# djukic14/BlockSparseMatrices.jl

Measured on AMD Instinct MI355X. Metric: fp64 block-SpMV GB/s (VBCRS mul!, algorithmic bytes / time), higher is better.
Workload: dtype f64

## Files before the change

### blocksparsematrices.jl_amd/csrc/bsm_analysis.cpp

```cpp
#include "bsm_analysis.h"

#include <algorithm>
#include <chrono>
#include <cstdio>
#include <cstdlib>
#include <cstring>
#include <numeric>
#include <set>
#include <thread>
#include <tuple>
#include <unordered_map>

namespace bsm {

Tunables Tunables::from_env() {
    Tunables t;
    auto geti = [](const char *name, int64_t dflt) -> int64_t {
        const char *s = std::getenv(name);
        if (!s || !*s) return dflt;
        return std::strtoll(s, nullptr, 10);
    };
    t.split2_bytes = geti("BSM_SPLIT2_BYTES", t.split2_bytes);
    t.split4_bytes = geti("BSM_SPLIT4_BYTES", t.split4_bytes);
    t.wgitem_max_bytes = geti("BSM_WGITEM_MAX_BYTES", t.wgitem_max_bytes);
    t.wave_bytes = geti("BSM_WAVE_BYTES", t.wave_bytes);
    t.multi_wave_bytes = geti("BSM_MULTI_WAVE_BYTES", t.multi_wave_bytes);
    t.target_waves = std::max<int64_t>(1, geti("BSM_TARGET_WAVES", t.target_waves));
    if (const char *f = std::getenv("BSM_FAT_FILL_BELOW")) t.fat_fill_below = std::atof(f);
    t.pack_threads = (int)geti("BSM_PACK_THREADS", t.pack_threads);
    t.wg_order = (int)geti("BSM_ORDER", t.wg_order);
    t.deep_group_bytes = geti("BSM_DEEP_GROUP_BYTES", t.deep_group_bytes);
    t.deep_total_bytes = geti("BSM_DEEP_TOTAL_BYTES", t.deep_total_bytes);
    t.window_bytes = (size_t)geti("BSM_UPLOAD_WINDOW_BYTES", (int64_t)t.window_bytes);
    if (t.pack_threads < 1) t.pack_threads = 1;
    return t;
}

namespace {

std::vector<std::vector<int32_t>> conflict_adjacency(const std::vector<const int64_t *> &lists,
                                                     const std::vector<int64_t> &lens) {
    const int64_t nb = (int64_t)lists.size();
    int64_t maxindex = 0;
    for (int64_t b = 0; b < nb; b++)
        for (int64_t k = 0; k < lens[b]; k++) maxindex = std::max(maxindex, lists[b][k]);
    std::vector<int64_t> ptr(maxindex + 2, 0);
    for (int64_t b = 0; b < nb; b++)
        for (int64_t k = 0; k < lens[b]; k++) ptr[lists[b][k] + 1]++;
    for (int64_t i = 0; i <= maxindex; i++) ptr[i + 1] += ptr[i];
    std::vector<int64_t> inc(ptr[maxindex + 1]);
    {
        std::vector<int64_t> fill(ptr.begin(), ptr.end() - 1);
        for (int64_t b = 0; b < nb; b++)
            for (int64_t k = 0; k < lens[b]; k++) inc[fill[lists[b][k]]++] = b;
    }
    std::vector<std::vector<int32_t>> adj(nb);
    std::vector<int64_t> stamp(nb, -1);
    for (int64_t v = 0; v < nb; v++) {
        stamp[v] = v;
        for (int64_t k = 0; k < lens[v]; k++) {
            int64_t i = lists[v][k];
            for (int64_t p = ptr[i]; p < ptr[i + 1]; p++) {
                int64_t w = inc[p];
// ... 204 lines not shown
        const int e_lo = (int)std::max<int64_t>(0, -w0);
        const int e_hi = (int)std::min<int64_t>(E, n - w0);
        U *d = dst + (s * mc) * E;
        if (!trans) {
            for (int e = e_lo; e < e_hi; e++) {
                const V *col = src + ra + (w0 + e) * ld;
                for (int i = 0; i < mc; i++) d[(int64_t)i * E + e] = stored(col[i]);
            }
        } else {
            for (int i = 0; i < mc; i++) {
                const V *row = src + w0 + (int64_t)(ra + i) * ld;
                for (int e = e_lo; e < e_hi; e++) d[(int64_t)i * E + e] = stored(row[e]);
            }
        }
    }
}

struct U16 {
    uint64_t a, b;
};

uint64_t hash_list(const int64_t *p, int64_t n) {
    uint64_t h = 0xcbf29ce484222325ull ^ (uint64_t)n;
    for (int64_t i = 0; i < n; i++) {
        h ^= (uint64_t)p[i];
        h *= 0x100000001b3ull;
        h ^= h >> 29;
    }
    return h;
}

}

struct Analysis::BuildState {
    bool sym = false;
    bool colored = false;
    int64_t nb = 0;
    int64_t own_lo = 0, own_hi = 0;
    std::vector<Chunk> chunks;
    std::vector<Group> groups;
    std::vector<const int64_t *> glist;
    std::vector<int32_t> colpos;
    std::vector<uint8_t> ckind;
    std::vector<uint8_t> group_perm;
    std::vector<int64_t> layout;
    uint64_t val_units = 0;
    std::vector<uint8_t> cover;
    std::vector<int32_t> group_color;
    int32_t ncolors_fused = 1;
    std::vector<Item> items;
    bool use_window = false;
};

std::string Analysis::build(int mtype_, int dtype_, int64_t nrows_, int64_t ncols_,
                            const std::vector<BlockIn> &blocks, const AnalysisOptions &opt_) {
    mtype = mtype_;
    dtype = dtype_;
    nrows = nrows_;
    ncols = ncols_;
    opt = opt_;
    tun = Tunables::from_env();
    const bool timing = std::getenv("BSM_TIMING") != nullptr;
    auto t_last = std::chrono::steady_clock::now();
    auto lap = [&](const char *what) {
        if (!timing) return;
        auto now = std::chrono::steady_clock::now();
        std::fprintf(stderr, "[bsm analysis] %-28s %8.1f ms\n", what,
                     std::chrono::duration<double, std::milli>(now - t_last).count());
        t_last = now;
    };
    BuildState st;
    std::string err = stage_validate(blocks, st);
    if (!err.empty()) return err;
    lap("validate");
    bool colour_oom = false;
    if (opt.meta_only) {
        reference_colourings(blocks, colour_oom);
        return colour_oom ? "out of host memory (colouring)" : "";
    }
    if (!(err = stage_row_groups(blocks, st)).empty()) return err;
    if (!(err = stage_merge_columns(blocks, st)).empty()) return err;
    lap("groups + column lists");
    if (!(err = stage_accumulation(blocks, st)).empty()) return err;
    lap("exclusivity / fused colours");
    std::thread colour_thread([&] { reference_colourings(blocks, colour_oom); });
    struct Joiner {
        std::thread &t;
        ~Joiner() {
            if (t.joinable()) t.join();
        }
    } colour_join{colour_thread};
    stage_work_items(st);
    stage_place_values(st);
    lap("work items + value placement");
    if (!(err = stage_pack_values(blocks, st)).empty()) return err;
    lap("pack values");
    stage_waves(st);
    stage_windows(st);
    if (!(err = stage_gather_index(st)).empty()) return err;
    lap("schedule");
    colour_thread.join();
    lap("reference colourings (tail not hidden by packing)");
    if (colour_oom) return "out of host memory (colouring)";
    return "";
}

std::string Analysis::stage_validate(const std::vector<BlockIn> &blocks, BuildState &st) {
    static const int kEs[6] = {4, 8, 8, 16, 4, 8};
    static const int kVs[6] = {4, 8, 8, 16, 8, 16};
    if (dtype < 0 || dtype > 5) return "unknown dtype";
    es = kEs[dtype];
    vs = kVs[dtype];
    E = 16 / es;
    if (nrows < 0 || ncols < 0) return "negative matrix size";
    if (nrows > INT32_MAX - 64 || ncols > INT32_MAX - 64) return "matrix dimension exceeds int32 range";
    const int64_t nb = st.nb = (int64_t)blocks.size();
    bool sym = (mtype == MT_SYMMETRIC);
    for (const BlockIn &B : blocks) sym |= (B.kind != KIND_PLAIN);
    st.sym = sym;
    st.own_lo = (opt.own_lo > 0) ? opt.own_lo - 1 : 0;
    st.own_hi = (opt.own_hi > 0) ? std::min(opt.own_hi, nrows) : nrows;
    const int64_t rlim = sym ? std::min(nrows, ncols) : nrows;
    const int64_t clim = sym ? std::min(nrows, ncols) : ncols;

    nnz = 0;
// ... 68 lines not shown
                }
            } else if (mtype == MT_SYMMETRIC) {
                std::vector<const int64_t *> dl, rl, cl;
                std::vector<int64_t> dn, rn, cn;
                for (const BlockIn &B : blocks) {
                    if (B.kind == KIND_DIAG) {
                        dl.push_back(B.ridx);
                        dn.push_back(B.ridx ? B.m : 0);
                    } else {
                        rl.push_back(B.ridx);
                        rn.push_back(B.ridx ? B.m : 0);
                        cl.push_back(B.cidx);
                        cn.push_back(B.cidx ? B.n : 0);
                    }
                }
                colors[0] = refcolor(rl, rn);
                colors[1] = refcolor(cl, cn);
                colors[2] = refcolor(dl, dn);
            }
        } catch (const std::bad_alloc &) {
            colour_oom = true;
        }
    }
}

std::string Analysis::stage_row_groups(const std::vector<BlockIn> &blocks, BuildState &st) {
    const int64_t nb = st.nb;
    auto &chunks = st.chunks;
    auto &groups = st.groups;
    auto &glist = st.glist;
    const int chunk_rows = tun.chunk_rows;
    std::unordered_map<uint64_t, std::vector<int64_t>> gmap;

    rows.clear();
    cols.clear();
    for (int64_t b = 0; b < nb; b++) {
        const BlockIn &B = blocks[b];
        if (B.m == 0 || B.n == 0) continue;
        for (int64_t ra = 0; ra < B.m; ra += chunk_rows) {
            const int mc = (int)std::min<int64_t>(chunk_rows, B.m - ra);
            bool rcontig = true;
            if (B.ridx)
                for (int i = 1; i < mc; i++)
                    if (B.ridx[ra + i] != B.ridx[ra] + i) {
                        rcontig = false;
                        break;
                    }
            const int64_t rbase = rcontig ? (B.ridx ? B.ridx[ra] : B.r0 + ra) - 1 : -1;
            uint64_t h;
            if (rcontig)
                h = ((uint64_t)rbase * 0x9E3779B97F4A7C15ull) ^ ((uint64_t)mc << 56) ^ 0x51ull;
            else
                h = hash_list(B.ridx + ra, mc);
            const int gkind = (B.kind == KIND_PLAIN) ? KIND_PLAIN : KIND_OFF;
            h ^= (uint64_t)gkind * 0xD6E8FEB86659FD93ull;
            int64_t gid = -1;
            auto &cand = gmap[h];
            for (int64_t g : cand) {
                const Group &G = groups[g];
                if (G.mc != mc || ((G.kind == KIND_PLAIN) != (B.kind == KIND_PLAIN))) continue;
                if (rcontig) {
                    if (G.rbase == rbase) gid = g;
                } else if (G.rbase < 0 &&
                           std::memcmp(glist[g], B.ridx + ra, sizeof(int64_t) * mc) == 0) {
                    gid = g;
                }
                if (gid >= 0) break;
            }
            if (gid < 0) {
                gid = (int64_t)groups.size();
                Group G;
                G.mc = mc;
                G.kind = B.kind;
                G.rbase = (int32_t)rbase;
                if (!rcontig) {
                    if ((int64_t)rows.size() + mc + 8 > INT32_MAX) return "row index pool exceeds int32";
                    G.row_off = (int32_t)rows.size();
                    for (int i = 0; i < mc; i++) rows.push_back((int32_t)(B.ridx[ra + i] - 1));
                }
                groups.push_back(G);
                glist.push_back(rcontig ? nullptr : B.ridx + ra);
                cand.push_back(gid);
            }
            Chunk c;
            c.blk = (int32_t)b;
            c.ra = (int32_t)ra;
            c.mc = mc;
            c.group = gid;
            c.woff = groups[gid].width;
            groups[gid].width += B.n;
            if (B.kind == KIND_OFF) {
                groups[gid].has_off = true;
                groups[gid].kind = KIND_OFF;
            } else if (B.kind == KIND_DIAG) {
                groups[gid].has_diag = true;
            }
            groups[gid].chunks.push_back((int32_t)chunks.size());
            chunks.push_back(c);
        }
    }
    ngroups = (int64_t)groups.size();
    return "";
}

std::string Analysis::stage_merge_columns(const std::vector<BlockIn> &blocks, BuildState &st) {
    auto &chunks = st.chunks;
    auto &groups = st.groups;
    auto &colpos = st.colpos;
    auto &ckind = st.ckind;
    auto &group_perm = st.group_perm;
    uint64_t val_units = 0;

    {
        int64_t total_cols = 0;
        for (const Group &G : groups) total_cols += G.width + E;
        if (total_cols + 8 > INT32_MAX) return "column index pool exceeds int32";
        cols.reserve((size_t)total_cols);
    }
    group_perm.assign(groups.size(), 0);
    colpos.reserve(cols.capacity());
    ckind.reserve(cols.capacity());
    {
        std::vector<int32_t> ord;
        size_t gi = 0;
        for (Group &G : groups) {
            G.strips = (G.width + E - 1) / E;
            if (G.strips * (int64_t)G.mc * 16 >= ((int64_t)1 << 31)) return "row group panel exceeds 2 GiB";
            G.col_off = (int64_t)cols.size();
            for (int32_t ci : G.chunks) {
                const BlockIn &B = blocks[chunks[ci].blk];
                for (int64_t k = 0; k < B.n; k++) {
                    cols.push_back((int32_t)((B.cidx ? B.cidx[k] : B.c0 + k) - 1));
                    ckind.push_back((uint8_t)B.kind);
                }
            }
            int32_t *gc = cols.data() + G.col_off;
            uint8_t *gk = ckind.data() + G.col_off;
            colpos.resize(cols.size());
            int32_t *gp = colpos.data() + G.col_off;
            if (std::is_sorted(gc, gc + G.width)) {
                for (int64_t q = 0; q < G.width; q++) gp[q] = (int32_t)q;
            } else {
                group_perm[gi] = 1;
                ord.resize((size_t)G.width);
                std::iota(ord.begin(), ord.end(), 0);
                std::stable_sort(ord.begin(), ord.end(), [&](int32_t a, int32_t b) { return gc[a] < gc[b]; });
                std::vector<int32_t> sorted((size_t)G.width);
                std::vector<uint8_t> sortedk((size_t)G.width);
                for (int64_t r = 0; r < G.width; r++) {
                    sorted[r] = gc[ord[r]];
                    sortedk[r] = gk[ord[r]];
                    gp[ord[r]] = (int32_t)r;
// ... 124 lines not shown
        if (tun.wgitem_max_bytes <= 0) tun.wgitem_max_bytes = 4 * W;
    }
    for (int64_t g = 0; g < ngroups; g++) {
        const Group &G = groups[g];
        const int64_t strip_bytes = (int64_t)G.mc * 16;
        int64_t per_item = G.strips;
        if (!exclusive_fwd && !colored) {
            int64_t maxs = std::max<int64_t>(1, tun.wgitem_max_bytes / strip_bytes);
            int64_t nitem = (G.strips + maxs - 1) / maxs;
            per_item = (G.strips + nitem - 1) / nitem;
        }
        for (int64_t s = 0; s < G.strips; s += per_item) {
            Item it;
            it.group = g;
            it.s_begin = s;
            it.s_end = std::min(G.strips, s + per_item);
            it.bytes = (it.s_end - it.s_begin) * strip_bytes;
            it.nw = it.bytes >= tun.split4_bytes ? 4 : (it.bytes >= tun.split2_bytes ? 2 : 1);
            it.color = group_color[g];
            items.push_back(it);
        }
    }
    const bool use_window = st.use_window = sym && !colored && !gather && !exclusive_fwd && tun.lds_window;
    auto locality = [&](const Item &it) -> int64_t {
        const Group &G = groups[it.group];
        return (G.rbase >= 0) ? G.rbase : rows[G.row_off];
    };
    std::stable_sort(items.begin(), items.end(), [&](const Item &a, const Item &b) {
        if (a.color != b.color) return a.color < b.color;
        if (a.nw != b.nw) return a.nw > b.nw;
        if (use_window && a.nw < 4) return locality(a) < locality(b);
        return a.bytes > b.bytes;
    });
}

void Analysis::stage_place_values(BuildState &st) {
    auto &groups = st.groups;
    std::vector<uint8_t> placed(groups.size(), 0);
    st.layout.clear();
    st.layout.reserve(groups.size());
    for (const Item &it : st.items)
        if (!placed[it.group]) {
            placed[it.group] = 1;
            st.layout.push_back(it.group);
        }
    for (size_t g = 0; g < groups.size(); g++)
        if (!placed[g]) st.layout.push_back((int64_t)g);
    uint64_t off = 0;
    for (int64_t g : st.layout) {
        groups[g].val_off = off;
        off += (uint64_t)groups[g].mc * (uint64_t)groups[g].strips;
    }
}

std::string Analysis::stage_pack_values(const std::vector<BlockIn> &blocks, BuildState &st) {
    auto &chunks = st.chunks;
    auto &groups = st.groups;
    auto &colpos = st.colpos;
    auto &group_perm = st.group_perm;
    const uint64_t val_units = st.val_units;

    auto pack_one = [&](const Chunk &c, char *dst) {
        const BlockIn &B = blocks[c.blk];
        if (group_perm[c.group]) {
            const int32_t *dp = colpos.data() + groups[c.group].col_off + c.woff;
            if (dtype == 4)
                pack_chunk_perm<float, double>((const double *)B.data, B.ld, c.ra, c.mc, B.n, dp, E, B.trans, (float *)dst);
            else if (dtype == 5)
                pack_chunk_perm<C64h, C128h>((const C128h *)B.data, B.ld, c.ra, c.mc, B.n, dp, E, B.trans, (C64h *)dst);
            else if (es == 4)
                pack_chunk_perm<uint32_t>((const uint32_t *)B.data, B.ld, c.ra, c.mc, B.n, dp, E, B.trans, (uint32_t *)dst);
            else if (es == 8)
                pack_chunk_perm<uint64_t>((const uint64_t *)B.data, B.ld, c.ra, c.mc, B.n, dp, E, B.trans, (uint64_t *)dst);
            else
                pack_chunk_perm<U16>((const U16 *)B.data, B.ld, c.ra, c.mc, B.n, dp, E, B.trans, (U16 *)dst);
            return;
        }
// ... 148 lines not shown
                            segx[nseg] = cols[G.col_off + k];
                            segk[nseg] = ckind[G.col_off + k];
                        }
                        nseg++;
                    }
                }
                if (nseg <= 3) {
                    P.xbase = segx[0];
                    W.seg1_w = segw[1];
                    W.seg1_x = segx[1];
                    W.seg2_w = segw[2];
                    P.seg2_x = segx[2];
                    P.kind = segk[0] | (segk[1] << 2) | (segk[2] << 4);
                } else {
                    P.xbase = -1;
                    W.seg1_w = W.seg2_w = P.ncols;
                    P.kind = G.kind;
                }
                if (piece_off) P.kind |= kKindHasOff;
                if (G.has_off) P.kind |= kKindGroupHasOff;
                W.npieces = 1;
            }
            waves.push_back(W);
        }
    };
    for (const Item &it : items) {
        if (colored && it.color != cur_color) {
            while (waves.size() % kWavesPerWg) emit_nop();
            while ((int32_t)color_wg_ptr.size() <= it.color)
                color_wg_ptr.push_back((int64_t)waves.size() / kWavesPerWg);
            cur_color = it.color;
        }
        item_waves(it);
    }
    while (waves.size() % kWavesPerWg) emit_nop();
    nwg_main = (int64_t)waves.size() / kWavesPerWg;
    const bool snake = tun.wg_order != 0 && exclusive_fwd;
    if (!colored && snake && nwg_main > 2) {
        std::vector<WaveWork> re(waves.size());
        const int64_t blk = 256;
        int64_t k = 0;
        for (int64_t a0 = 0; a0 < nwg_main; a0 += blk) {
            const int64_t a1 = std::min(nwg_main, a0 + blk);
            for (int64_t j = 0; j < a1 - a0; j++, k++) {
                const int64_t src = ((a0 / blk) & 1) ? a1 - 1 - j : a0 + j;
                for (int w = 0; w < kWavesPerWg; w++) re[k * kWavesPerWg + w] = waves[src * kWavesPerWg + w];
            }
        }
        waves.swap(re);
    }
    if (colored) {
        while ((int32_t)color_wg_ptr.size() <= ncolors_fused) color_wg_ptr.push_back(nwg_main);
    }

    if (exclusive_fwd) {
        int64_t r = own_lo;
        while (r < own_hi) {
            if (cover[r]) {
                r++;
                continue;
            }
            int64_t e = r;
            while (e < own_hi && !cover[e] && e - r < kScaleRowsPerWave) e++;
            WaveWork W;
            std::memset(&W, 0, sizeof W);
            W.work = WORK_SCALE;
            W.grp = 1;
            W.rbase = (int32_t)r;
            W.first.ncols = (int32_t)(e - r);
            waves.push_back(W);
            r = e;
// ... 211 lines not shown
```

### blocksparsematrices.jl_amd/csrc/bsm_analysis.h

```cpp
#pragma once
#include <cstdint>
#include <string>
#include <vector>

#include "bsm_layout.h"

namespace bsm {

class RawBuffer {
  public:
    RawBuffer() = default;
    RawBuffer(const RawBuffer &) = delete;
    RawBuffer &operator=(const RawBuffer &) = delete;
    ~RawBuffer() { release(); }
    void allocate(size_t n) {
        release();
        p_ = n ? static_cast<char *>(::operator new(n)) : nullptr;
        n_ = n;
    }
    void release() {
        if (p_) ::operator delete(p_);
        p_ = nullptr;
        n_ = 0;
    }
// ... 6 lines not shown
  private:
    char *p_ = nullptr;
    size_t n_ = 0;
};

enum MatType { MT_VBCRS = 0, MT_BLOCKSPARSE = 1, MT_SYMMETRIC = 2 };

struct BlockIn {
    const char *data;
    int64_t m, n, ld;
    const int64_t *ridx;
    const int64_t *cidx;
    int64_t r0, c0;
    int kind;
    bool trans = false;
};

struct Tunables {
    int64_t wave_bytes = 0;
    int64_t target_waves = 32768;
    double fat_fill_below = 0.9;
    int64_t wave_bytes_min = 8 << 10, wave_bytes_max = 24 << 10;
    int64_t multi_wave_bytes = 64 << 10;
    int64_t split2_bytes = 0;
    int64_t split4_bytes = 0;
    int64_t wgitem_max_bytes = 0;
    int chunk_rows = kMaxRowsPerChunk;
    int64_t deep_group_bytes = 128 << 10;
    int64_t deep_total_bytes = 64 << 20;
    int pack_threads = 8;
    size_t window_bytes = 64u << 20;
    int lds_window = 1;
    int wg_order = -1;
    static Tunables from_env();
};

struct ValueSink {
    virtual ~ValueSink() = default;
    virtual std::string begin(size_t total_bytes, bool *use) = 0;
    virtual char *window(size_t bytes) = 0;
    virtual std::string commit(size_t offset, size_t bytes) = 0;
    virtual std::string end() = 0;
};

struct AnalysisOptions {
    int scheduler = 0;
    int validate = 1;
    int accumulate = 0;
    int64_t own_lo = 0, own_hi = 0;
    ValueSink *sink = nullptr;
    bool blocks_on_device = false;
    int coloring = 0;
    bool meta_only = false;
    bool skip_colors = false;
};

std::vector<std::vector<int64_t>> color_dsatur(const std::vector<const int64_t *> &lists,
                                               const std::vector<int64_t> &lens);
std::vector<std::vector<int64_t>> color_workstream_dsatur(const std::vector<const int64_t *> &lists,
                                                          const std::vector<int64_t> &lens);

struct PackChunk {
    uint64_t src;
    uint64_t dst_unit;
    int64_t ld;
    int32_t ra, mc;
    int32_t n, woff;
    int32_t perm_off;
    int32_t trans;
};
static_assert(sizeof(PackChunk) == 48, "PackChunk must be 48 bytes");

class Analysis {
  public:
    int mtype = 0, dtype = 0;
    int es = 8;
    int vs = 8;
    int E = 2;
    int64_t nrows = 0, ncols = 0;
    AnalysisOptions opt;
    Tunables tun;

    std::vector<int64_t> perm, rowptr, colindices, rowindices;
    std::vector<std::vector<int64_t>> colors[3];
    int64_t nnz = 0, stored_entries = 0, alg_bytes = 0;

    RawBuffer values;
    std::vector<PackChunk> pack_plan;
    std::vector<int32_t> pack_colpos;
    int64_t value_bytes = 0;
    std::vector<int32_t> rows, cols;
    std::vector<WaveWork> waves;
    std::vector<WaveWork> waves_multi;
    int64_t nwg_multi = 0;
    double lane_fill = 1.0;
    double mean_rows = 64.0;
    int64_t nwg_main = 0;
    int64_t nwg_total = 0;
    int64_t ngroups = 0;
    bool exclusive_fwd = false;
    std::vector<int64_t> color_wg_ptr;
    int64_t win_emissions = 0, win_inside = 0, win_flushed = 0;
    bool gather = false;
    int64_t ws_fbase = 0, ws_slots = 0;
    std::vector<int64_t> inv_ptr[2];
    std::vector<int32_t> inv_idx[2];

    std::string build(int mtype, int dtype, int64_t nrows, int64_t ncols,
                      const std::vector<BlockIn> &blocks, const AnalysisOptions &opt);

    std::vector<int64_t> vbcrs_bookkeeping(int64_t nblocks, const int64_t *rowstart, const int64_t *colstart);

  private:
    struct BuildState;
    std::string stage_validate(const std::vector<BlockIn> &blocks, BuildState &st);
    void reference_colourings(const std::vector<BlockIn> &blocks, bool &colour_oom);
    std::string stage_row_groups(const std::vector<BlockIn> &blocks, BuildState &st);
    std::string stage_merge_columns(const std::vector<BlockIn> &blocks, BuildState &st);
    std::string stage_accumulation(const std::vector<BlockIn> &blocks, BuildState &st);
    void stage_work_items(BuildState &st);
    void stage_place_values(BuildState &st);
    std::string stage_pack_values(const std::vector<BlockIn> &blocks, BuildState &st);
    void stage_waves(BuildState &st);
    void stage_windows(BuildState &st);
    std::string stage_gather_index(BuildState &st);
};

}
```

### blocksparsematrices.jl_amd/csrc/bsm_device.h

```cpp
#pragma once
#include <hip/hip_runtime.h>

#include <cstdlib>
#include <type_traits>

#include "../../include/bsm_rocm.h"
#include "bsm_analysis.h"
#include "bsm_kernels.h"
#include "bsm_layout.h"

namespace bsm {

struct c64 {
    float re, im;
};
struct c128 {
    double re, im;
};

template <typename T> struct TT;
template <> struct TT<float> {
    static constexpr int E = 4;
};
template <> struct TT<double> {
// ... 157 lines not shown
}

template <typename T, int V, int P> struct Butterfly {
    static constexpr int half(int cur) { return cur >= 2 ? cur / 2 : 1; }
    static __device__ __forceinline__ void run(T *v, int i, int &pos, int &dup) {
        constexpr int C0 = V;
        constexpr int C1 = (P >= 16) ? half(C0) : C0;
        constexpr int C2 = half(C1);
        constexpr int C3 = half(C2);
        constexpr int C4 = half(C3);
        constexpr int C5 = (P >= 32) ? half(C4) : C4;
        if constexpr (P >= 16) bfly_step<T, C0, 8>(v, i, pos, dup, [](T a) { return dppx<DPP_ROW_MIRROR>(a); });
        bfly_step<T, C1, 4>(v, i, pos, dup, [](T a) { return dppx<DPP_ROW_HALF_MIRROR>(a); });
        bfly_step<T, C2, 2>(v, i, pos, dup, [](T a) { return dppx<DPP_QUAD_XOR3>(a); });
        bfly_step<T, C3, 1>(v, i, pos, dup, [](T a) { return dppx<DPP_QUAD_XOR1>(a); });
        if constexpr (P >= 32) bfly_step<T, C4, 16>(v, i, pos, dup, [](T a) { return shx(a, 16); });
        if constexpr (P >= 64) bfly_step<T, C5, 32>(v, i, pos, dup, [](T a) { return shx(a, 32); });
    }
};

template <typename T, int CUR, int D> struct ReduceAbove {
    static __device__ __forceinline__ void run(T *v, int lane, int &pos, int &dup) {
        if constexpr (D < 64) {
            bfly_step<T, CUR, D>(v, lane, pos, dup, [](T a) { return shx(a, D); });
            ReduceAbove<T, (CUR >= 2 ? CUR / 2 : 1), D * 2>::run(v, lane, pos, dup);
        }
    }
};

#ifdef BSM_TRACE
static __device__ unsigned long long *g_trace = nullptr;
static hipError_t set_trace_here(void *buf) { return hipMemcpyToSymbol(HIP_SYMBOL(g_trace), &buf, sizeof(buf)); }
__shared__ unsigned long long t_trace[kWavesPerWg][16];
#define BSM_TSTAMP(slot)                                                   \
    do {                                                                   \
        if (lane == 0) t_trace[threadIdx.x >> 6][(slot)] = clock64();      \
    } while (0)
#else
#define BSM_TSTAMP(slot) \
    do {                 \
    } while (0)
#endif

constexpr int FLAG_STRONG_ZERO = 1;
constexpr int FLAG_DIRECT = 2;
constexpr int FLAG_CONJ = 4;
constexpr int FLAG_OPT = 8;
constexpr int FLAG_RMW = 16;
constexpr int FLAG_GATHER = 32;
constexpr int FLAG_KACT_SHIFT = 8;
#ifdef BSM_EXPERIMENT
constexpr int DBG_NO_GLOBAL_ATOMICS = 1 << 16;
constexpr int DBG_NO_WINDOW_ADD = 1 << 17;
constexpr int DBG_NO_BUTTERFLY = 1 << 18;
constexpr int DBG_NO_EMISSION = 1 << 19;
constexpr int DBG_NO_XGATHER = 1 << 20;
constexpr int DBG_NO_FWD_OUT = 1 << 21;
constexpr int DBG_NO_MATRIX = 1 << 22;
constexpr int DBG_NO_FWD_HALF = 1 << 23;
constexpr int DBG_NO_TRN_HALF = 1 << 24;
#define BSM_DBG(bit) ((flags & (bit)) != 0)
#else
#define BSM_DBG(bit) false
#endif

struct PieceD {
    uint32_t val_lo, val_hi;
// ... 158 lines not shown
```

### blocksparsematrices.jl_amd/csrc/bsm_one.hip

```cpp
#include "bsm_device.h"
#include "bsm_families.h"

namespace bsm {

#ifndef BSM_C64_FUSED_WAVES
#define BSM_C64_FUSED_WAVES 5
#endif
#ifndef BSM_C128_FUSED_WAVES
#define BSM_C128_FUSED_WAVES 6
#endif

template <typename T, int L, int P, bool FWD, bool TRN, bool NT, typename S = T>
__device__ __forceinline__ T run_panel(const WaveD &wd, const uint4 *__restrict__ values,
                                       const int *__restrict__ rows, const int *__restrict__ cols,
                                       const T *__restrict__ x, T *__restrict__ y, T alpha,
                                       int flags, int lane, T *xs, T *vs, T *win, int win_n,
                                       T *__restrict__ ws) {
    constexpr int E = TT<S>::E;
    constexpr int G = 64 / P;
    constexpr int V = L * E;
    constexpr int NC = G * L * E;
    constexpr int XCH = x_chunk_cols<T, TRN>();
    using XV = typename std::conditional<std::is_same<S, T>::value, Vec16<T>, XVec<T, E>>::type;
    constexpr int BF = XCH / NC;
// ... 213 lines not shown

template <typename T, int L, bool FWD, bool TRN, bool NT, typename S = T>
__global__ void __launch_bounds__(64 * kWavesPerWg) __attribute__((amdgpu_waves_per_eu(
    kCvec<T, S> ? BSM_CVEC_WAVES :
    !std::is_same<S, T>::value ? kMixedWaves<T, FWD, TRN> :
    (FWD && TRN && (std::is_same<T, double>::value || std::is_same<T, float>::value)) ? 8 :
    (FWD && TRN && std::is_same<T, c128>::value) ? (L == 4 ? 8 : BSM_C128_FUSED_WAVES) :
    (FWD && TRN && std::is_same<T, c64>::value) ? (L == 4 ? 8 : BSM_C64_FUSED_WAVES) :
    (((!TRN && std::is_same<T, double>::value) || std::is_same<T, c128>::value) ? 6 : 5))))
    __attribute__((amdgpu_num_sgpr(96)))
    panel_kernel(const WaveWork *__restrict__ waves, const uint4 *__restrict__ values, const int *__restrict__ rows,
                 const int *__restrict__ cols, const T *__restrict__ x, T *__restrict__ y, T alpha,
                 T beta, int flags, unsigned wg_base, T *__restrict__ ws, long long ws_fbase) {
    constexpr int XS = x_chunk_cols<T, TRN>();
    constexpr int VS = XS;
    __shared__ __attribute__((aligned(16))) T xs[kWavesPerWg][FWD ? XS : 1];
    __shared__ __attribute__((aligned(16))) T vs[kWavesPerWg][TRN ? VS : 1];
    constexpr bool WIN = FWD && TRN;
    __shared__ T win[WIN ? window_entries((int)sizeof(T)) : 1];

    const int wave = __builtin_amdgcn_readfirstlane(threadIdx.x >> 6);
    const int lane = threadIdx.x & 63;
    BSM_TSTAMP(0);
    const WaveD wd = load_wave(waves + ((size_t)(blockIdx.x + wg_base) * kWavesPerWg + wave));
    const int work = wd.work;
    const int m = wd.m;
#ifdef BSM_TRACE
    asm volatile("s_waitcnt lgkmcnt(0)" ::: "memory");
    BSM_TSTAMP(1);
    if (lane == 0) {
        t_trace[threadIdx.x >> 6][6] =
            (unsigned long long)(wd.work == WORK_PANEL && wd.npieces ? (long long)wd.first.nstrips * wd.m * 16 : 0);
        t_trace[threadIdx.x >> 6][7] = wall_clock64();
    }
#endif
    int win_n = (WIN && !(flags & FLAG_RMW)) ? wd.win_n : 0;
    if constexpr (kCvec<T, S>) win_n = min(win_n, window_entries((int)sizeof(T)));
    if (WIN && win_n > 0) {
        for (int e = threadIdx.x; e < win_n; e += 64 * kWavesPerWg) win[e] = zero_of(T{});
        __syncthreads();
    }

    T u = zero_of(T{});
    if (work == WORK_PANEL) {
        if (m <= 8)
            u = run_panel<T, L, 8, FWD, TRN, NT, S>(wd, values, rows, cols, x, y, alpha, flags, lane, xs[wave], vs[wave], win, win_n, ws);
        else if (m <= 16)
            u = run_panel<T, L, 16, FWD, TRN, NT, S>(wd, values, rows, cols, x, y, alpha, flags, lane, xs[wave], vs[wave], win, win_n, ws);
        else if (m <= 32)
            u = run_panel<T, L, 32, FWD, TRN, NT, S>(wd, values, rows, cols, x, y, alpha, flags, lane, xs[wave], vs[wave], win, win_n, ws);
        else
            u = run_panel<T, L, 64, FWD, TRN, NT, S>(wd, values, rows, cols, x, y, alpha, flags, lane, xs[wave], vs[wave], win, win_n, ws);
    }
    BSM_TSTAMP(4);
    const bool direct = (flags & FLAG_DIRECT) != 0;
    const bool sz = (flags & FLAG_STRONG_ZERO) != 0;
    if (FWD) {
        if (wd.wg_sync) {
            xs[wave][lane] = u;
            __syncthreads();
        }
        if (work == WORK_PANEL && wd.lead && !BSM_DBG(DBG_NO_FWD_OUT)) {
            for (int k = 1; k < wd.grp; ++k) u = add(u, xs[wave + k][lane]);
            if (flags & FLAG_GATHER) {
                const bool fwd_on = !(flags & FLAG_OPT) || (wd.first.kind & kKindGroupHasOff);
                if (lane < m && fwd_on) ws[ws_fbase + wd.win_base + lane] = u;
// ... 185 lines not shown
```

### blocksparsematrices.jl_amd/csrc/bsm_operator.cpp

```cpp
#include <hip/hip_runtime_api.h>

#include <algorithm>
#include <climits>
#include <cstdlib>
#include <cstring>
#include <mutex>
#include <string>
#include <vector>

#include "bsm_internal.h"

namespace bsm {

namespace {

template <typename V> hipError_t upload(const V &v, void **dptr, long long &total) {
    const size_t bytes = v.size() * sizeof(decltype(v[0]));
    hipError_t e = hipMalloc(dptr, bytes ? bytes : 16);
    if (e != hipSuccess) return e;
    total += (long long)bytes;
    if (bytes) e = hipMemcpy(*dptr, v.data(), bytes, hipMemcpyHostToDevice);
    return e;
}

// ... 637 lines not shown
    return BSM_OK;
}

bool capturing(hipStream_t st) {
    hipStreamCaptureStatus cs = hipStreamCaptureStatusNone;
    if (hipStreamIsCapturing(st, &cs) != hipSuccess) {
        (void)hipGetLastError();
        return false;
    }
    return cs != hipStreamCaptureStatusNone;
}

AnalysisOptions to_aopt(const bsm_options &o, ValueSink *sink) {
    AnalysisOptions a;
    a.sink = sink;
    a.blocks_on_device = (o.blocks_memspace == BSM_MEM_DEVICE);
    a.coloring = (int)o.coloring;
    a.scheduler = o.scheduler;
    a.validate = 1;
    a.accumulate = o.accumulate;
    a.own_lo = o.own_lo;
    a.own_hi = o.own_hi;
    return a;
}

int LocalOperator::build(int mtype, int dtype, int64_t nrows, int64_t ncols, const std::vector<BlockIn> &in,
                         const std::vector<int64_t> &ids, int64_t nids, const bsm_options &o, bool colors, const std::string &prefix) {
    const bool devblocks = (o.blocks_memspace == BSM_MEM_DEVICE);
    if (devblocks && device == BSM_DEVICE_NONE) return fail(BSM_ERR_INVALID, "device-resident blocks need a device handle");
    const bool streamed = device != BSM_DEVICE_NONE && !devblocks;
    DeviceSink sink(&img.d_values), sink_t(&img_t.d_values);
    AnalysisOptions ao = to_aopt(o, streamed ? &sink : nullptr);
    ao.skip_colors = !colors;
    std::string err = an.build(mtype, dtype, nrows, ncols, in, ao);
    ao.sink = nullptr;
    bool want_t = o.transpose_image == 1;
    if (o.transpose_image == 2 && device != BSM_DEVICE_NONE) {
        size_t free_b = 0, total_b = 0;
        if (hipMemGetInfo(&free_b, &total_b) == hipSuccess)
            want_t = (size_t)an.value_bytes <= free_b / 16;
        else
            (void)hipGetLastError();
    }
    AnalysisOptions ao_t = transpose_aopt(o);
    if (err.empty() && want_t && mtype != MT_SYMMETRIC) {
        bool plain = true;
        for (const BlockIn &B : in) plain &= (B.kind == KIND_PLAIN);
        if (plain) {
            ao_t.sink = streamed ? &sink_t : nullptr;
            err = an_t.build(MT_BLOCKSPARSE, an.dtype, an.ncols, an.nrows, transposed_blocks(in), ao_t);
            ao_t.sink = nullptr;
            has_t = err.empty();
        }
    }
    if (!err.empty()) return build_error(prefix + err);
    upd_in = keep_inputs(mtype, dtype, nrows, ncols, in, ids, nids, ao, has_t ? &ao_t : nullptr);
    if (devblocks) {
        hipError_t e = device_pack(an, &img.d_values);
        if (e == hipSuccess && has_t) e = device_pack(an_t, &img_t.d_values);
        if (e != hipSuccess) return hip_fail(e, "device-side packing");
    }
    fill_image(an, o, true, img);
    if (has_t) fill_image(an_t, o, false, img_t);
    if (device != BSM_DEVICE_NONE) {
        hipError_t e = upload_image(an, img, device);
        if (e == hipSuccess && has_t) e = upload_image(an_t, img_t, device);
        if (e != hipSuccess) return hip_fail(e, "device upload");
    }
    return BSM_OK;
}

void LocalOperator::release() {
    free_image(img);
    free_image(img_t);
    update_free(upd);
    il_free(il);
}
// ... 18 lines not shown
```

Baseline: 5735.

## Cut oversized row groups and balance workgroup dispatch order across CUs

Adds a planning pass that splits heavy plain row groups into shorter row cuts when the whole launch fits in resident workgroup capacity, then rebuilds groups and work items. Adds a dispatch-order stage that assigns workgroups to CU slots by greedy LPT plus pairwise swaps, and lays out packed values in that order. The aim is to shrink the tail caused by a few heavy workgroups on one CU. It assumes round-robin dispatch to CUs and adds extra analysis time and a second grouping pass; it also adds hardware-ID trace fields for debugging.

```diff
diff --git a/blocksparsematrices.jl_amd/csrc/bsm_analysis.cpp b/blocksparsematrices.jl_amd/csrc/bsm_analysis.cpp
--- a/blocksparsematrices.jl_amd/csrc/bsm_analysis.cpp
+++ b/blocksparsematrices.jl_amd/csrc/bsm_analysis.cpp
@@ -1,7 +1,9 @@
 #include "bsm_analysis.h"
 
 #include <algorithm>
+#include <cassert>
 #include <chrono>
+#include <cmath>
 #include <cstdio>
 #include <cstdlib>
 #include <cstring>
@@ -29,6 +31,8 @@
     if (const char *f = std::getenv("BSM_FAT_FILL_BELOW")) t.fat_fill_below = std::atof(f);
     t.pack_threads = (int)geti("BSM_PACK_THREADS", t.pack_threads);
     t.wg_order = (int)geti("BSM_ORDER", t.wg_order);
+    t.wg_cap_pct = (int)geti("BSM_WG_CAP", t.wg_cap_pct);
+    t.resident_wgs = geti("BSM_RESIDENT_WGS", t.resident_wgs);
     t.deep_group_bytes = geti("BSM_DEEP_GROUP_BYTES", t.deep_group_bytes);
     t.deep_total_bytes = geti("BSM_DEEP_TOTAL_BYTES", t.deep_total_bytes);
     t.window_bytes = (size_t)geti("BSM_UPLOAD_WINDOW_BYTES", (int64_t)t.window_bytes);
@@ -299,6 +303,10 @@
 
 }
 
+namespace {
+int64_t count_scale_waves(const std::vector<uint8_t> &cover, int64_t own_lo, int64_t own_hi);
+}
+
 struct Analysis::BuildState {
     bool sym = false;
     bool colored = false;
@@ -317,6 +325,10 @@
     int32_t ncolors_fused = 1;
     std::vector<Item> items;
     bool use_window = false;
+    std::unordered_map<uint64_t, int32_t> cuts;
+    std::vector<int64_t> item_wg;
+    int64_t nwg_items = 0;
+    std::vector<int64_t> wg_perm;
 };
 
 std::string Analysis::build(int mtype_, int dtype_, int64_t nrows_, int64_t ncols_,
@@ -358,6 +370,15 @@
         }
     } colour_join{colour_thread};
     stage_work_items(st);
+    if (plan_cuts(st)) {
+        if (!(err = stage_row_groups(blocks, st)).empty()) return err;
+        if (!(err = stage_merge_columns(blocks, st)).empty()) return err;
+        if (!(err = stage_accumulation(blocks, st)).empty()) return err;
+        stage_work_items(st);
+        assert(st.nwg_items + (count_scale_waves(st.cover, st.own_lo, st.own_hi) + kWavesPerWg - 1) / kWavesPerWg <= resident_capacity());
+        lap("row cuts: groups again");
+    }
+    stage_dispatch_order(st);
     stage_place_values(st);
     lap("work items + value placement");
     if (!(err = stage_pack_values(blocks, st)).empty()) return err;
@@ -492,71 +513,88 @@
     const int chunk_rows = tun.chunk_rows;
     std::unordered_map<uint64_t, std::vector<int64_t>> gmap;
 
+    chunks.clear();
+    groups.clear();
+    glist.clear();
     rows.clear();
     cols.clear();
     for (int64_t b = 0; b < nb; b++) {
         const BlockIn &B = blocks[b];
         if (B.m == 0 || B.n == 0) continue;
-        for (int64_t ra = 0; ra < B.m; ra += chunk_rows) {
-            const int mc = (int)std::min<int64_t>(chunk_rows, B.m - ra);
-            bool rcontig = true;
-            if (B.ridx)
-                for (int i = 1; i < mc; i++)
-                    if (B.ridx[ra + i] != B.ridx[ra] + i) {
-                        rcontig = false;
-                        break;
+        for (int64_t ra0 = 0; ra0 < B.m; ra0 += chunk_rows) {
+            const int mc0 = (int)std::min<int64_t>(chunk_rows, B.m - ra0);
+            int cut_h = mc0;
+            if (!st.cuts.empty() && B.kind == KIND_PLAIN) {
+                bool contig = true;
+                if (B.ridx)
+                    for (int i = 1; i < mc0 && contig; i++) contig = B.ridx[ra0 + i] == B.ridx[ra0] + i;
+                if (contig) {
+                    const int64_t rb = (B.ridx ? B.ridx[ra0] : B.r0 + ra0) - 1;
+                    auto it = st.cuts.find(((uint64_t)rb << 8) | (uint64_t)mc0);
+                    if (it != st.cuts.end()) cut_h = it->second;
+                }
+            }
+            for (int64_t ra = ra0; ra < ra0 + mc0; ra += cut_h) {
+                const int mc = (int)std::min<int64_t>(cut_h, ra0 + mc0 - ra);
+                bool rcontig = true;
+                if (B.ridx)
+                    for (int i = 1; i < mc; i++)
+                        if (B.ridx[ra + i] != B.ridx[ra] + i) {
+                            rcontig = false;
+                            break;
+                        }
+                const int64_t rbase = rcontig ? (B.ridx ? B.ridx[ra] : B.r0 + ra) - 1 : -1;
+                uint64_t h;
+                if (rcontig)
+                    h = ((uint64_t)rbase * 0x9E3779B97F4A7C15ull) ^ ((uint64_t)mc << 56) ^ 0x51ull;
+                else
+                    h = hash_list(B.ridx + ra, mc);
+                const int gkind = (B.kind == KIND_PLAIN) ? KIND_PLAIN : KIND_OFF;
+                h ^= (uint64_t)gkind * 0xD6E8FEB86659FD93ull;
+                int64_t gid = -1;
+                auto &cand = gmap[h];
+                for (int64_t g : cand) {
+                    const Group &G = groups[g];
+                    if (G.mc != mc || ((G.kind == KIND_PLAIN) != (B.kind == KIND_PLAIN))) continue;
+                    if (rcontig) {
+                        if (G.rbase == rbase) gid = g;
+                    } else if (G.rbase < 0 &&
+                               std::memcmp(glist[g], B.ridx + ra, sizeof(int64_t) * mc) == 0) {
+                        gid = g;
                     }
-            const int64_t rbase = rcontig ? (B.ridx ? B.ridx[ra] : B.r0 + ra) - 1 : -1;
-            uint64_t h;
-            if (rcontig)
-                h = ((uint64_t)rbase * 0x9E3779B97F4A7C15ull) ^ ((uint64_t)mc << 56) ^ 0x51ull;
-            else
-                h = hash_list(B.ridx + ra, mc);
-            const int gkind = (B.kind == KIND_PLAIN) ? KIND_PLAIN : KIND_OFF;
-            h ^= (uint64_t)gkind * 0xD6E8FEB86659FD93ull;
-            int64_t gid = -1;
-            auto &cand = gmap[h];
-            for (int64_t g : cand) {
-                const Group &G = groups[g];
-                if (G.mc != mc || ((G.kind == KIND_PLAIN) != (B.kind == KIND_PLAIN))) continue;
-                if (rcontig) {
-                    if (G.rbase == rbase) gid = g;
-                } else if (G.rbase < 0 &&
-                           std::memcmp(glist[g], B.ridx + ra, sizeof(int64_t) * mc) == 0) {
-                    gid = g;
+                    if (gid >= 0) break;
                 }
-                if (gid >= 0) break;
-            }
-            if (gid < 0) {
-                gid = (int64_t)groups.size();
-                Group G;
-                G.mc = mc;
-                G.kind = B.kind;
-                G.rbase = (int32_t)rbase;
-                if (!rcontig) {
-                    if ((int64_t)rows.size() + mc + 8 > INT32_MAX) return "row index pool exceeds int32";
-                    G.row_off = (int32_t)rows.size();
-                    for (int i = 0; i < mc; i++) rows.push_back((int32_t)(B.ridx[ra + i] - 1));
+                if (gid < 0) {
+                    gid = (int64_t)groups.size();
+                    Group G;
+                    G.mc = mc;
+                    G.kind = B.kind;
+                    G.rbase = (int32_t)rbase;
+                    if (!rcontig) {
+                        if ((int64_t)rows.size() + mc + 8 > INT32_MAX) return "row index pool exceeds int32";
+                        G.row_off = (int32_t)rows.size();
+                        for (int i = 0; i < mc; i++) rows.push_back((int32_t)(B.ridx[ra + i] - 1));
+                    }
+                    groups.push_back(G);
+                    glist.push_back(rcontig ? nullptr : B.ridx + ra);
+                    cand.push_back(gid);
                 }
-                groups.push_back(G);
-                glist.push_back(rcontig ? nullptr : B.ridx + ra);
-                cand.push_back(gid);
-            }
-            Chunk c;
-            c.blk = (int32_t)b;
-            c.ra = (int32_t)ra;
-            c.mc = mc;
-            c.group = gid;
-            c.woff = groups[gid].width;
-            groups[gid].width += B.n;
-            if (B.kind == KIND_OFF) {
-                groups[gid].has_off = true;
-                groups[gid].kind = KIND_OFF;
-            } else if (B.kind == KIND_DIAG) {
-                groups[gid].has_diag = true;
-            }
-            groups[gid].chunks.push_back((int32_t)chunks.size());
-            chunks.push_back(c);
+                Chunk c;
+                c.blk = (int32_t)b;
+                c.ra = (int32_t)ra;
+                c.mc = mc;
+                c.group = gid;
+                c.woff = groups[gid].width;
+                groups[gid].width += B.n;
+                if (B.kind == KIND_OFF) {
+                    groups[gid].has_off = true;
+                    groups[gid].kind = KIND_OFF;
+                } else if (B.kind == KIND_DIAG) {
+                    groups[gid].has_diag = true;
+                }
+                groups[gid].chunks.push_back((int32_t)chunks.size());
+                chunks.push_back(c);
+            }
         }
     }
     ngroups = (int64_t)groups.size();
@@ -578,6 +616,8 @@
         cols.reserve((size_t)total_cols);
     }
     group_perm.assign(groups.size(), 0);
+    colpos.clear();
+    ckind.clear();
     colpos.reserve(cols.capacity());
     ckind.reserve(cols.capacity());
     {
@@ -768,6 +808,132 @@
         if (use_window && a.nw < 4) return locality(a) < locality(b);
         return a.bytes > b.bytes;
     });
+    st.item_wg.clear();
+    st.nwg_items = 0;
+    if (!colored) {
+        int64_t pos = 0;
+        for (const Item &it : items) {
+            while ((pos % kWavesPerWg) % it.nw != 0) pos++;
+            st.item_wg.push_back(pos / kWavesPerWg);
+            pos += it.nw;
+        }
+        st.nwg_items = (pos + kWavesPerWg - 1) / kWavesPerWg;
+    }
+}
+
+int64_t Analysis::resident_capacity() const {
+    if (tun.resident_wgs > 0) return tun.resident_wgs;
+    const int64_t cus = opt.num_cus > 0 ? opt.num_cus : 256;
+    const int64_t waves_per_simd = (dtype == 0 || dtype == 2) ? 5 : 6;
+    return cus * 4 * waves_per_simd / kWavesPerWg;
+}
+
+namespace {
+int64_t count_scale_waves(const std::vector<uint8_t> &cover, int64_t own_lo, int64_t own_hi) {
+    int64_t n = 0, r = own_lo;
+    while (r < own_hi) {
+        if (cover[r]) {
+            r++;
+            continue;
+        }
+        int64_t e = r;
+        while (e < own_hi && !cover[e] && e - r < kScaleRowsPerWave) e++;
+        n++;
+        r = e;
+    }
+    return n;
+}
+}
+
+bool Analysis::plan_cuts(BuildState &st) {
+    st.cuts.clear();
+    if (tun.wg_cap_pct <= 0 || !exclusive_fwd || st.colored || gather || st.sym) return false;
+    int64_t nwaves = 0, bytes = 0;
+    for (const Item &it : st.items) {
+        nwaves += it.nw;
+        bytes += it.bytes;
+    }
+    const int64_t scale_wgs = (count_scale_waves(st.cover, st.own_lo, st.own_hi) + kWavesPerWg - 1) / kWavesPerWg;
+    const int64_t nwg = st.nwg_items, capacity = resident_capacity();
+    if (nwg < 2 || nwg + scale_wgs > capacity) return false;
+    auto waves_of = [&](int64_t b) { return b >= tun.split4_bytes ? 4 : (b >= tun.split2_bytes ? 2 : 1); };
+    double cap = (double)bytes / (double)nwg * tun.wg_cap_pct / 100.0;
+    for (int attempt = 0; attempt < 64; attempt++, cap *= 1.1) {
+        st.cuts.clear();
+        int64_t extra = 0;
+        for (const Item &it : st.items) {
+            const Group &G = st.groups[it.group];
+            if (it.nw < kWavesPerWg || (double)it.bytes <= cap || G.rbase < 0 || G.kind != KIND_PLAIN || G.mc < 16) continue;
+            const int64_t k = (int64_t)std::ceil((double)it.bytes / cap);
+            const int h = (int)std::max<int64_t>(8, ((G.mc + k - 1) / k + 7) / 8 * 8);
+            if (h >= G.mc) continue;
+            for (int r = 0; r < G.mc; r += h) extra += waves_of((int64_t)std::min(h, G.mc - r) * G.strips * 16);
+            extra -= it.nw;
+            st.cuts[((uint64_t)G.rbase << 8) | (uint64_t)G.mc] = h;
+        }
+        if (st.cuts.empty()) return false;
+        if ((nwaves + extra + kWavesPerWg - 1) / kWavesPerWg + scale_wgs <= capacity) return true;
+    }
+    st.cuts.clear();
+    return false;
+}
+
+static int64_t dispatch_cu(int64_t slot, int64_t ncus) { return slot % ncus; }
+
+void Analysis::stage_dispatch_order(BuildState &st) {
+    st.wg_perm.clear();
+    const int order = tun.wg_order < 0 ? 2 : tun.wg_order;
+    if (order != 2 || !exclusive_fwd || st.colored) return;
+    const int64_t nwg = st.nwg_items;
+    std::vector<int64_t> cost((size_t)nwg, 0);
+    for (size_t i = 0; i < st.items.size(); i++) cost[(size_t)st.item_wg[i]] += st.items[i].bytes;
+    const int64_t scale_wgs = (count_scale_waves(st.cover, st.own_lo, st.own_hi) + kWavesPerWg - 1) / kWavesPerWg;
+    if (nwg < 3 || nwg + scale_wgs > resident_capacity()) return;
+    const int64_t ncus = std::min<int64_t>(nwg, opt.num_cus > 0 ? opt.num_cus : 256);
+    std::vector<std::vector<int64_t>> slots((size_t)ncus);
+    for (int64_t k = 0; k < nwg; k++) slots[(size_t)dispatch_cu(k, ncus)].push_back(k);
+    std::vector<int64_t> by_cost((size_t)nwg);
+    std::iota(by_cost.begin(), by_cost.end(), 0);
+    std::stable_sort(by_cost.begin(), by_cost.end(), [&](int64_t a, int64_t b) { return cost[a] > cost[b]; });
+    using Load = std::pair<int64_t, int64_t>;
+    std::set<Load> open;
+    for (int64_t c = 0; c < ncus; c++)
+        if (!slots[(size_t)c].empty()) open.insert(Load(0, c));
+    std::vector<std::vector<int64_t>> mine((size_t)ncus);
+    std::vector<int64_t> load((size_t)ncus, 0);
+    for (int64_t w : by_cost) {
+        const Load l = *open.begin();
+        open.erase(open.begin());
+        const size_t c = (size_t)l.second;
+        mine[c].push_back(w);
+        load[c] += cost[w];
+        if (mine[c].size() < slots[c].size()) open.insert(Load(load[c], l.second));
+    }
+    for (int64_t round = 0; round < 8 * ncus; round++) {
+        const size_t a = (size_t)(std::max_element(load.begin(), load.end()) - load.begin());
+        int64_t best = load[a];
+        size_t bc = 0, bi = 0, bj = 0;
+        for (size_t c = 0; c < (size_t)ncus; c++) {
+            if (c == a) continue;
+            for (size_t i = 0; i < mine[a].size(); i++)
+                for (size_t j = 0; j < mine[c].size(); j++) {
+                    const int64_t d = cost[mine[a][i]] - cost[mine[c][j]];
+                    if (d <= 0) continue;
+                    const int64_t worst = std::max(load[a] - d, load[c] + d);
+                    if (worst < best) best = worst, bc = c, bi = i, bj = j;
+                }
+        }
+        if (best == load[a]) break;
+        const int64_t d = cost[mine[a][bi]] - cost[mine[bc][bj]];
+        std::swap(mine[a][bi], mine[bc][bj]);
+        load[a] -= d;
+        load[bc] += d;
+    }
+    st.wg_perm.assign((size_t)nwg, -1);
+    for (size_t c = 0; c < (size_t)ncus; c++) {
+        std::stable_sort(mine[c].begin(), mine[c].end(), [&](int64_t a, int64_t b) { return cost[a] > cost[b]; });
+        for (size_t i = 0; i < mine[c].size(); i++) st.wg_perm[(size_t)slots[c][i]] = mine[c][i];
+    }
 }
 
 void Analysis::stage_place_values(BuildState &st) {
@@ -775,10 +941,19 @@
     std::vector<uint8_t> placed(groups.size(), 0);
     st.layout.clear();
     st.layout.reserve(groups.size());
-    for (const Item &it : st.items)
-        if (!placed[it.group]) {
-            placed[it.group] = 1;
-            st.layout.push_back(it.group);
+    std::vector<const Item *> order;
+    order.reserve(st.items.size());
+    if (st.wg_perm.empty()) {
+        for (const Item &it : st.items) order.push_back(&it);
+    } else {
+        std::vector<std::vector<const Item *>> of_wg(st.wg_perm.size());
+        for (size_t i = 0; i < st.items.size(); i++) of_wg[(size_t)st.item_wg[i]].push_back(&st.items[i]);
+        for (int64_t w : st.wg_perm) order.insert(order.end(), of_wg[(size_t)w].begin(), of_wg[(size_t)w].end());
+    }
+    for (const Item *it : order)
+        if (!placed[it->group]) {
+            placed[it->group] = 1;
+            st.layout.push_back(it->group);
         }
     for (size_t g = 0; g < groups.size(); g++)
         if (!placed[g]) st.layout.push_back((int64_t)g);
@@ -993,11 +1168,19 @@
             cur_color = it.color;
         }
         item_waves(it);
+        assert(colored || (int64_t)(waves.size() - (size_t)it.nw) / kWavesPerWg == st.item_wg[(size_t)(&it - items.data())]);
     }
     while (waves.size() % kWavesPerWg) emit_nop();
     nwg_main = (int64_t)waves.size() / kWavesPerWg;
+    assert(colored || nwg_main == st.nwg_items);
     const bool snake = tun.wg_order != 0 && exclusive_fwd;
-    if (!colored && snake && nwg_main > 2) {
+    if (!st.wg_perm.empty()) {
+        assert((int64_t)st.wg_perm.size() == nwg_main);
+        std::vector<WaveWork> re(waves.size());
+        for (int64_t k = 0; k < nwg_main; k++)
+            for (int w = 0; w < kWavesPerWg; w++) re[k * kWavesPerWg + w] = waves[st.wg_perm[k] * kWavesPerWg + w];
+        waves.swap(re);
+    } else if (!colored && snake && nwg_main > 2) {
         std::vector<WaveWork> re(waves.size());
         const int64_t blk = 256;
         int64_t k = 0;
diff --git a/blocksparsematrices.jl_amd/csrc/bsm_analysis.h b/blocksparsematrices.jl_amd/csrc/bsm_analysis.h
--- a/blocksparsematrices.jl_amd/csrc/bsm_analysis.h
+++ b/blocksparsematrices.jl_amd/csrc/bsm_analysis.h
@@ -62,6 +62,8 @@
     size_t window_bytes = 64u << 20;
     int lds_window = 1;
     int wg_order = -1;
+    int wg_cap_pct = 150;
+    int64_t resident_wgs = 0;
     static Tunables from_env();
 };
 
@@ -83,6 +85,7 @@
     int coloring = 0;
     bool meta_only = false;
     bool skip_colors = false;
+    int num_cus = 0;
 };
 
 std::vector<std::vector<int64_t>> color_dsatur(const std::vector<const int64_t *> &lists,
@@ -149,6 +152,9 @@
     std::string stage_merge_columns(const std::vector<BlockIn> &blocks, BuildState &st);
     std::string stage_accumulation(const std::vector<BlockIn> &blocks, BuildState &st);
     void stage_work_items(BuildState &st);
+    int64_t resident_capacity() const;
+    bool plan_cuts(BuildState &st);
+    void stage_dispatch_order(BuildState &st);
     void stage_place_values(BuildState &st);
     std::string stage_pack_values(const std::vector<BlockIn> &blocks, BuildState &st);
     void stage_waves(BuildState &st);
diff --git a/blocksparsematrices.jl_amd/csrc/bsm_device.h b/blocksparsematrices.jl_amd/csrc/bsm_device.h
--- a/blocksparsematrices.jl_amd/csrc/bsm_device.h
+++ b/blocksparsematrices.jl_amd/csrc/bsm_device.h
@@ -213,7 +213,9 @@
 static __device__ unsigned long long *g_trace = nullptr;
 static hipError_t set_trace_here(void *buf) { return hipMemcpyToSymbol(HIP_SYMBOL(g_trace), &buf, sizeof(buf)); }
 __shared__ unsigned long long t_trace[kWavesPerWg][16];
-#define BSM_TSTAMP(slot)                                                   \
+#define BSM_GETREG_HW_ID (4 | (31 << 11))
+#define BSM_GETREG_XCC_ID (20 | (31 << 11))
+#define BSM_TSTAMP(slot)                                                  \
     do {                                                                   \
         if (lane == 0) t_trace[threadIdx.x >> 6][(slot)] = clock64();      \
     } while (0)
diff --git a/blocksparsematrices.jl_amd/csrc/bsm_one.hip b/blocksparsematrices.jl_amd/csrc/bsm_one.hip
--- a/blocksparsematrices.jl_amd/csrc/bsm_one.hip
+++ b/blocksparsematrices.jl_amd/csrc/bsm_one.hip
@@ -269,6 +269,8 @@
         t_trace[threadIdx.x >> 6][6] =
             (unsigned long long)(wd.work == WORK_PANEL && wd.npieces ? (long long)wd.first.nstrips * wd.m * 16 : 0);
         t_trace[threadIdx.x >> 6][7] = wall_clock64();
+        t_trace[threadIdx.x >> 6][9] = (unsigned long long)__builtin_amdgcn_s_getreg(BSM_GETREG_HW_ID);
+        t_trace[threadIdx.x >> 6][10] = (unsigned long long)__builtin_amdgcn_s_getreg(BSM_GETREG_XCC_ID);
     }
 #endif
     int win_n = (WIN && !(flags & FLAG_RMW)) ? wd.win_n : 0;
diff --git a/blocksparsematrices.jl_amd/csrc/bsm_operator.cpp b/blocksparsematrices.jl_amd/csrc/bsm_operator.cpp
--- a/blocksparsematrices.jl_amd/csrc/bsm_operator.cpp
+++ b/blocksparsematrices.jl_amd/csrc/bsm_operator.cpp
@@ -693,6 +693,13 @@
     DeviceSink sink(&img.d_values), sink_t(&img_t.d_values);
     AnalysisOptions ao = to_aopt(o, streamed ? &sink : nullptr);
     ao.skip_colors = !colors;
+    if (device != BSM_DEVICE_NONE) {
+        int ncu = 0;
+        if (hipDeviceGetAttribute(&ncu, hipDeviceAttributeMultiprocessorCount, device) == hipSuccess)
+            ao.num_cus = ncu;
+        else
+            (void)hipGetLastError();
+    }
     std::string err = an.build(mtype, dtype, nrows, ncols, in, ao);
     ao.sink = nullptr;
     bool want_t = o.transpose_image == 1;
@@ -704,6 +711,7 @@
             (void)hipGetLastError();
     }
     AnalysisOptions ao_t = transpose_aopt(o);
+    ao_t.num_cus = ao.num_cus;
     if (err.empty() && want_t && mtype != MT_SYMMETRIC) {
         bool plain = true;
         for (const BlockIn &B : in) plain &= (B.kind == KIND_PLAIN);
```

New measurement: 6150, median of 6. +7.2%, better.
